# daovietanh190499/3D_Reconstruction

Measured on AMD Instinct MI355X. Metric: image-pairs matched/sec, higher is better.
Workload: dtype f32 descriptors: int8 MFMA certified filter + f64 re-score; 1 GPU; C3/C4 all-pairs BF-L2 + ratio 0.75: 257 imgs x 4096 kpts x 256-d, exact f32-input semantics (oracle.match.bf_match_exact, bit for bit); pairs=32896, api=dist.match_all_pairs_sharded(exact=True), match_mode=exact-float, parallelism=pairs/1

## Files before the change

### 3d_reconstruction_amd/csrc/match_exact.hip

```cpp
#include "match_dev.h"
#include "resolve_scratch.h"

namespace sfmhip {

__global__ __launch_bounds__(256) void desc_residual_kernel(const float* __restrict__ x, const int8_t* __restrict__ q,
                                                            int n_rows, int m_pad, int d, const int32_t* __restrict__ nk,
                                                            int mode, double* __restrict__ erow,
                                                            unsigned long long* __restrict__ eimg) {
    const int lane = threadIdx.x & 63;
    const int row = blockIdx.x * 4 + (threadIdx.x >> 6);
    if (row >= n_rows) return;
    const int img = row / m_pad, r = row % m_pad;
    if (r >= nk[img]) {
        if (lane == 0) erow[row] = 0.0;
        return;
    }
    const float* xr = x + (size_t)row * d;
    const int8_t* qr = q + (size_t)row * d;
    double s2 = 0.0, x2 = 0.0, v2 = 0.0;
    bool finite = true;
    for (int k = lane; k < d; k += 64) {
        const float xf = xr[k];
        const double xv = (double)xf;
        const double v = mode == 0 ? (double)((int)qr[k] + 128) : (double)qr[k] / 127.0;
        const double dl = xv - v;
        s2 = __builtin_fma(dl, dl, s2);
        x2 = __builtin_fma(xv, xv, x2);
        v2 = __builtin_fma(v, v, v2);
        finite = finite && __builtin_isfinite(xf);
    }
#pragma unroll
    for (int off = 32; off >= 1; off >>= 1) {
        s2 += __shfl_xor(s2, off);
        x2 += __shfl_xor(x2, off);
        v2 += __shfl_xor(v2, off);
    }
    const bool all_finite = __all(finite);
    if (lane == 0) {
        const double e = all_finite ? sqrt(s2) * (1.0 + 0x1p-40) + 0x1p-50 * (sqrt(x2) + sqrt(v2)) * (1.0 + 0x1p-40)
                                    : __builtin_inf();
        erow[row] = e;
        atomicMax(eimg + img, (unsigned long long)__double_as_longlong(e));
    }
}

constexpr int kResolveCap = 512;
#ifdef SFMHIP_RESOLVE_PROF
__device__ unsigned long long g_rprof[16];
#endif
template <int D, typename OutT>
__device__ __forceinline__ void resolve_row(int64_t e, int mark, const int8_t* __restrict__ q,
                                            const float* __restrict__ x, const int32_t* __restrict__ nk, int m_pad,
                                            const int32_t* __restrict__ pairs, const double* __restrict__ erow,
                                            const double* __restrict__ eimg, double s, double rn2, double rd2,
                                            OutT* __restrict__ m0, unsigned* __restrict__ n_resolved, float* sxa,
                                            int* sqa, int* scand, int lane) {
    constexpr int W4 = D / 4;
    const int pair = (int)(e / m_pad), i = (int)(e % m_pad);
    const int a = pairs[2 * pair], b = pairs[2 * pair + 1], nb = nk[b];
    const size_t arow = (size_t)a * m_pad + i;
    for (int k = lane; k < D; k += 64) sxa[k] = x[arow * D + k];
    for (int w = lane; w < W4; w += 64) sqa[w] = reinterpret_cast<const int*>(q + arow * D)[w];
    __builtin_amdgcn_fence(__ATOMIC_RELEASE, "wavefront");
    __builtin_amdgcn_wave_barrier();
    __builtin_amdgcn_fence(__ATOMIC_ACQUIRE, "wavefront");
    int na = 0;
    for (int w = lane; w < W4; w += 64) na = __builtin_amdgcn_sdot4(sqa[w], sqa[w], na, false);
#pragma unroll
    for (int off = 32; off >= 1; off >>= 1) na += __shfl_xor(na, off);
    const double se = (erow[arow] + eimg[b]) * s * (1.0 + 1e-12);
    const double bq = (se + (mark_sqrt_d2<OutT>(mark) + se) * (1.0 + 1e-12)) * (1.0 + 1e-12);
    const double tq = floor(bq * bq) + 1.0;
    int ncand = 0;
    for (int j0 = 0; j0 < nb; j0 += 64) {
        const int j = j0 + lane;
        bool in = false;
        if (j < nb) {
            const int4* qb = reinterpret_cast<const int4*>(q + ((size_t)b * m_pad + j) * D);
            int dot = 0, nbn = 0;
#pragma unroll 4
            for (int w4 = 0; w4 < W4 / 4; ++w4) {
                const int4 t = qb[w4];
                const int4 u = reinterpret_cast<const int4*>(sqa)[w4];
                dot = __builtin_amdgcn_sdot4(t.x, u.x, dot, false);
                dot = __builtin_amdgcn_sdot4(t.y, u.y, dot, false);
                dot = __builtin_amdgcn_sdot4(t.z, u.z, dot, false);
                dot = __builtin_amdgcn_sdot4(t.w, u.w, dot, false);
                nbn = __builtin_amdgcn_sdot4(t.x, t.x, nbn, false);
                nbn = __builtin_amdgcn_sdot4(t.y, t.y, nbn, false);
                nbn = __builtin_amdgcn_sdot4(t.z, t.z, nbn, false);
                nbn = __builtin_amdgcn_sdot4(t.w, t.w, nbn, false);
            }
            in = (double)((long long)na + nbn - 2LL * dot) <= tq;
        }
        const unsigned long long cb = __ballot(in);
        const int pos = ncand + __popcll(cb & ((1ull << lane) - 1ull));
        if (in && pos < kResolveCap) scand[pos] = j;
        ncand += __popcll(cb);
    }
    __builtin_amdgcn_fence(__ATOMIC_RELEASE, "wavefront");
    __builtin_amdgcn_wave_barrier();
    __builtin_amdgcn_fence(__ATOMIC_ACQUIRE, "wavefront");
    const bool every = ncand > kResolveCap;
    const int nc = every ? nb : ncand;
    double v1 = __builtin_inf(), v2 = __builtin_inf();
    int j1 = INT_MAX;
    for (int t = lane; t < nc; t += 64) {
        const int j = every ? t : scand[t];
        const float4* xb = reinterpret_cast<const float4*>(x + ((size_t)b * m_pad + j) * D);
        double acc = 0.0;
        for (int k4 = 0; k4 < D / 4; ++k4) {
            const float4 xv = xb[k4];
            double df;
            df = (double)sxa[4 * k4] - (double)xv.x;
            acc = acc + df * df;
            df = (double)sxa[4 * k4 + 1] - (double)xv.y;
            acc = acc + df * df;
            df = (double)sxa[4 * k4 + 2] - (double)xv.z;
            acc = acc + df * df;
            df = (double)sxa[4 * k4 + 3] - (double)xv.w;
            acc = acc + df * df;
        }
        if (acc < v1) { v2 = v1; v1 = acc; j1 = j; }
        else if (acc < v2) v2 = acc;
    }
#pragma unroll
    for (int off = 32; off >= 1; off >>= 1) {
        const double o1 = __shfl_xor(v1, off), o2 = __shfl_xor(v2, off);
        const int oj = __shfl_xor(j1, off);
        const bool mine = v1 < o1 || (v1 == o1 && j1 < oj);
        const double n2 = mine ? fmin(v2, o1) : fmin(o2, v1);
        if (!mine) { v1 = o1; j1 = oj; }
        v2 = n2;
    }
    const double p1 = rd2 * v1, e1 = __builtin_fma(rd2, v1, -p1);
    const double p2 = rn2 * v2, e2 = __builtin_fma(rn2, v2, -p2);
    const bool acc_ok = p1 < p2 || (p1 == p2 && e1 < e2);
    if (lane == 0) {
        m0[e] = (OutT)(acc_ok ? j1 : -1);
        if (n_resolved) atomicAdd(n_resolved, 1u);
    }
    __builtin_amdgcn_wave_barrier();
}

template <int D, typename OutT>
__global__ __launch_bounds__(256) void match_resolve_kernel(const int8_t* __restrict__ q, const float* __restrict__ x,
                                                            const int32_t* __restrict__ nk, int m_pad,
                                                            const int32_t* __restrict__ pairs, int P,
                                                            const double* __restrict__ erow,
                                                            const double* __restrict__ eimg, double s, double rn2,
                                                            double rd2, OutT* __restrict__ m0,
                                                            unsigned* __restrict__ n_resolved,
                                                            const unsigned* __restrict__ overflow = nullptr) {
    if (overflow && *overflow == 0u) return;
    constexpr int W4 = D / 4;
    __shared__ float sxa[4][D];
    __shared__ __attribute__((aligned(16))) int sqa[4][W4];
    __shared__ int scand[4][kResolveCap];
    const int lane = threadIdx.x & 63, wave = threadIdx.x >> 6;
    const int64_t total = (int64_t)P * m_pad;
    const int64_t nchunk = (total + 63) >> 6;
    for (int64_t c = (int64_t)blockIdx.x * 4 + wave; c < nchunk; c += (int64_t)gridDim.x * 4) {
        const int64_t e0 = c << 6;
        const int v = (e0 + lane < total) ? (int)m0[e0 + lane] : -1;
        unsigned long long bal = __ballot(v <= kUndecidedBase);
        while (bal) {
            const int l = __builtin_ctzll(bal);
            bal &= bal - 1;
            resolve_row<D, OutT>(e0 + l, __shfl(v, l), q, x, nk, m_pad, pairs, erow, eimg, s, rn2, rd2, m0, n_resolved,
                           sxa[wave], sqa[wave], scand[wave], lane);
        }
    }
}

template <typename OutT>
__global__ __launch_bounds__(256) void resolve_collect_kernel(const OutT* __restrict__ m0, int64_t total, int m_pad,
                                                              const int32_t* __restrict__ pairs,
                                                              unsigned* __restrict__ cnt, int64_t* __restrict__ list,
                                                              unsigned* __restrict__ overflow) {
    auto take = [&](int64_t e) {
        const int b = pairs[2 * (int)(e / m_pad) + 1];
        const unsigned slot = atomicAdd(cnt + b, 1u);
        if (slot < (unsigned)kResolveBucket) list[(size_t)b * kResolveBucket + slot] = e;
        else atomicOr(overflow, 1u);
    };
    constexpr int PER = 16 / sizeof(OutT);
    const int64_t n4 = total / PER;
    const int4* m4 = reinterpret_cast<const int4*>(m0);
    for (int64_t e4 = (int64_t)blockIdx.x * blockDim.x + threadIdx.x; e4 < n4; e4 += (int64_t)gridDim.x * blockDim.x) {
        const int4 v = m4[e4];
        if constexpr (sizeof(OutT) == 2) {
            const unsigned w[4] = {(unsigned)v.x, (unsigned)v.y, (unsigned)v.z, (unsigned)v.w};
            bool any = false;
#pragma unroll
            for (int h = 0; h < 4; ++h) {
                any |= (short)(w[h] & 0xFFFFu) <= kUndecidedBase;
                any |= (short)(w[h] >> 16) <= kUndecidedBase;
            }
            if (!any) continue;
#pragma unroll
            for (int h = 0; h < 4; ++h) {
                if ((short)(w[h] & 0xFFFFu) <= kUndecidedBase) take(PER * e4 + 2 * h);
                if ((short)(w[h] >> 16) <= kUndecidedBase) take(PER * e4 + 2 * h + 1);
            }
        } else {
            if (min(min(v.x, v.y), min(v.z, v.w)) > kUndecidedBase) continue;
            if (v.x <= kUndecidedBase) take(4 * e4);
            if (v.y <= kUndecidedBase) take(4 * e4 + 1);
            if (v.z <= kUndecidedBase) take(4 * e4 + 2);
            if (v.w <= kUndecidedBase) take(4 * e4 + 3);
        }
    }
}

__global__ __launch_bounds__(1024) void resolve_offsets_kernel(
    const unsigned* __restrict__ cnt, int n_img, unsigned* __restrict__ off, unsigned* __restrict__ okey,
    int* __restrict__ oimg, unsigned* __restrict__ xr, int* __restrict__ items, unsigned* __restrict__ ir,
    const unsigned* __restrict__ overflow) {
    __shared__ unsigned sr[1024], sk[1024];
    __shared__ unsigned sxs[9], sks[9];
    if (*overflow != 0u) return;
    const int tid = threadIdx.x;
    const int cap = n_img * (kResolveBucket / kResolveRows + 1);
    int ps[9];
    ps[0] = 0;
#pragma unroll
    for (int x = 0; x < 8; ++x) ps[x + 1] = ps[x] + (x < n_img ? (n_img - x + 7) / 8 : 0);
    unsigned carry_r = 0, carry_k = 0;
    for (int base = 0; base < n_img; base += 1024) {
        const int p = base + tid;
        int b = -1;
        unsigned cb = 0, ni = 0;
        if (p < n_img) {
            int x = 0;
#pragma unroll
            for (int y = 1; y < 8; ++y) x += (p >= ps[y]) ? 1 : 0;
            b = x + 8 * (p - ps[x]);
            cb = min(cnt[b], (unsigned)kResolveBucket);
            ni = (cb + kResolveRows - 1) / kResolveRows;
        }
        sr[tid] = cb;
        sk[tid] = ni;
        __syncthreads();
        for (int d = 1; d < 1024; d <<= 1) {
            const unsigned vr = tid >= d ? sr[tid - d] : 0u, vk = tid >= d ? sk[tid - d] : 0u;
            __syncthreads();
            sr[tid] += vr;
            sk[tid] += vk;
            __syncthreads();
        }
        const unsigned run = carry_r + sr[tid] - cb, k0 = carry_k + sk[tid] - ni;
        if (b >= 0) {
            off[b] = run;
            okey[p] = run;
            oimg[p] = b;
#pragma unroll
            for (int x = 0; x < 8; ++x)
                if (p == ps[x]) {
                    sxs[x] = run;
                    sks[x] = k0;
                }
            for (unsigned i = 0; i < ni; ++i) {
                items[k0 + i] = (int)(run + i * kResolveRows);
                items[cap + k0 + i] = (int)min((unsigned)kResolveRows, cb - i * kResolveRows);
                items[2 * cap + k0 + i] = b;
            }
        }
        carry_r += sr[1023];
        carry_k += sk[1023];
        __syncthreads();
    }
    if (tid < 9) {
        if (tid == 8 || ps[tid] >= n_img) {
            sxs[tid] = carry_r;
            sks[tid] = carry_k;
        }
    }
    __syncthreads();
    if (tid < 8) {
        xr[tid] = sxs[tid];
        xr[8 + tid] = sxs[tid + 1] - sxs[tid];
        ir[tid] = sks[tid];
        ir[8 + tid] = sks[tid + 1] - sks[tid];
    }
    if (tid == 0) okey[n_img] = carry_r;
}
__global__ __launch_bounds__(256) void resolve_flatten_kernel(const unsigned* __restrict__ okey,
                                                              const int* __restrict__ oimg, int n_img,
                                                              const int64_t* __restrict__ list,
                                                              int64_t* __restrict__ flat,
                                                              const unsigned* __restrict__ overflow) {
    if (*overflow != 0u) return;
    const unsigned total = okey[n_img];
    for (unsigned t = blockIdx.x * blockDim.x + threadIdx.x; t < total; t += gridDim.x * blockDim.x) {
        int lo = 0, hi = n_img - 1;
        while (lo < hi) {
            const int mid = (lo + hi + 1) >> 1;
            if (okey[mid] <= t) lo = mid;
            else hi = mid - 1;
        }
        flat[t] = list[(size_t)oimg[lo] * kResolveBucket + (t - okey[lo])];
    }
}

template <int D, typename OutT>
__global__ __launch_bounds__(256) void match_resolve_batched_kernel(
    const int8_t* __restrict__ q , const int32_t* __restrict__ norms,
    const float* __restrict__ x, const int32_t* __restrict__ nk, int m_pad,
    const int32_t* __restrict__ pairs, int n_img, const double* __restrict__ erow, const double* __restrict__ eimg,
    double s, double rn2, double rd2, OutT* __restrict__ m0, unsigned* __restrict__ n_resolved,
    const int64_t* __restrict__ flat, const int* __restrict__ items, const unsigned* __restrict__ ir,
    const unsigned* __restrict__ overflow) {
    constexpr int W4 = D / 4, R = kResolveRows;
    __shared__ __attribute__((aligned(16))) int sqa[R][W4];
    __shared__ float sxa[R][D];
    __shared__ int scand[R][kResolveCap];
    __shared__ int sncand[R], sna[R], sccd[R];
    __shared__ double stq[R];
    __shared__ int64_t se_[R];
    if (*overflow != 0u) return;
    const int tid = threadIdx.x, lane = tid & 63, wave = tid >> 6;
    const int cap = n_img * (kResolveBucket / kResolveRows + 1);
    const int xcd = blockIdx.x % 8, nx = (gridDim.x + 7 - xcd) / 8;
    const unsigned ib = ir[xcd], in = ir[8 + xcd];
    for (unsigned k = blockIdx.x / 8; k < in; k += nx) {
        const int f0 = items[ib + k], nr = items[cap + ib + k], b = items[2 * cap + ib + k];
        const int nb = nk[b];
        for (int t = tid; t < nr * W4; t += 256) {
            const int r = t / W4, w = t % W4;
            const int64_t e = flat[f0 + r];
            const size_t arow = (size_t)pairs[2 * (int)(e / m_pad)] * m_pad + (int)(e % m_pad);
            sqa[r][w] = reinterpret_cast<const int*>(q + arow * D)[w];
        }
        for (int t = tid; t < nr * D; t += 256) {
            const int r = t / D, kk = t % D;
            const int64_t e = flat[f0 + r];
            const size_t arow = (size_t)pairs[2 * (int)(e / m_pad)] * m_pad + (int)(e % m_pad);
            sxa[r][kk] = x[arow * D + kk];
        }
        if (tid < R) sncand[tid] = 0;
        __syncthreads();
        for (int r = wave; r < nr; r += 4) {
            int na = 0;
            for (int w = lane; w < W4; w += 64) na = __builtin_amdgcn_sdot4(sqa[r][w], sqa[r][w], na, false);
#pragma unroll
            for (int off = 32; off >= 1; off >>= 1) na += __shfl_xor(na, off);
            if (lane == 0) {
                const int64_t e = flat[f0 + r];
                const size_t arow = (size_t)pairs[2 * (int)(e / m_pad)] * m_pad + (int)(e % m_pad);
                const double se = (erow[arow] + eimg[b]) * s * (1.0 + 1e-12);
                const double bq = (se + (mark_sqrt_d2<OutT>((int)m0[e]) + se) * (1.0 + 1e-12)) * (1.0 + 1e-12);
                stq[r] = floor(bq * bq) + 1.0;
                sna[r] = na;
                sccd[r] = norms[arow] - na;
                se_[r] = e;
            }
        }
        __syncthreads();
        {
            using M16 = Mfma<16>;
            constexpr int KK = D / M16::KB;
            const int lr = lane & 15, grp = lane >> 4;
            i32x4 bqv[KK];
#pragma unroll
            for (int kk = 0; kk < KK; ++kk) bqv[kk] = *reinterpret_cast<const i32x4*>(&sqa[lr][kk * 16 + grp * 4]);
            const bool live = lr < nr;
            const long long na_r = live ? (long long)sna[lr] - sccd[lr] : 0;
            const double tq_r = live ? stq[lr] : -1.0;
            const size_t bbase = (size_t)b * m_pad;
            constexpr int TG = 4;
            for (int jg = wave * 16; jg < nb; jg += 64 * TG) {
                i32x4 av[TG][KK], nv[TG];
#pragma unroll
                for (int t = 0; t < TG; ++t) {
                    const int j0 = min(jg + 64 * t, m_pad - 16);
                    const int8_t* rp = q + (bbase + j0 + lr) * D + grp * 16;
#pragma unroll
                    for (int kk = 0; kk < KK; ++kk) av[t][kk] = *reinterpret_cast<const i32x4*>(rp + kk * M16::KB);
                    nv[t] = *reinterpret_cast<const i32x4*>(norms + bbase + j0 + 4 * grp);
                }
#pragma unroll
                for (int t = 0; t < TG; ++t) {
                    const int j0 = jg + 64 * t;
                    i32x4 acc = {0, 0, 0, 0};
#pragma unroll
                    for (int kk = 0; kk < KK; ++kk) acc = M16::run(av[t][kk], bqv[kk], acc);
#pragma unroll
                    for (int e = 0; e < 4; ++e) {
                        const int j = j0 + 4 * grp + e;
                        if (live && j < nb && (double)(na_r + nv[t][e] - 2LL * acc[e]) <= tq_r) {
                            const int pos = atomicAdd(&sncand[lr], 1);
                            if (pos < kResolveCap) scand[lr][pos] = j;
                        }
                    }
                }
            }
        }
        __syncthreads();
        for (int r = wave; r < nr; r += 4) {
            const int ncand = sncand[r];
            const bool every = ncand > kResolveCap;
#ifdef SFMHIP_RESOLVE_PROF
            if (lane == 0) {
                atomicAdd(&g_rprof[0], 1ull);
                atomicAdd(&g_rprof[1], (unsigned long long)ncand);
                if (every) atomicAdd(&g_rprof[2], 1ull);
                atomicMax(&g_rprof[3], (unsigned long long)ncand);
                atomicAdd(&g_rprof[4 + min(ncand / 64, 11)], 1ull);
            }
#endif
            const int nc = every ? nb : ncand;
            double v1 = __builtin_inf(), v2 = __builtin_inf();
            int j1 = INT_MAX;
            for (int t = lane; t < nc; t += 64) {
                const int j = every ? t : scand[r][t];
                const float4* xb = reinterpret_cast<const float4*>(x + ((size_t)b * m_pad + j) * D);
                double acc = 0.0;
                for (int k4 = 0; k4 < D / 4; ++k4) {
                    const float4 xv = xb[k4];
                    double df;
                    df = (double)sxa[r][4 * k4] - (double)xv.x;
                    acc = acc + df * df;
                    df = (double)sxa[r][4 * k4 + 1] - (double)xv.y;
                    acc = acc + df * df;
                    df = (double)sxa[r][4 * k4 + 2] - (double)xv.z;
                    acc = acc + df * df;
                    df = (double)sxa[r][4 * k4 + 3] - (double)xv.w;
                    acc = acc + df * df;
                }
                if (acc < v1 || (acc == v1 && j < j1)) { v2 = v1; v1 = acc; j1 = j; }
                else if (acc < v2) v2 = acc;
            }
#pragma unroll
            for (int off = 32; off >= 1; off >>= 1) {
                const double o1 = __shfl_xor(v1, off), o2 = __shfl_xor(v2, off);
                const int oj = __shfl_xor(j1, off);
                const bool mine = v1 < o1 || (v1 == o1 && j1 < oj);
                const double n2 = mine ? fmin(v2, o1) : fmin(o2, v1);
                if (!mine) { v1 = o1; j1 = oj; }
                v2 = n2;
            }
            const double p1 = rd2 * v1, e1 = __builtin_fma(rd2, v1, -p1);
            const double p2 = rn2 * v2, e2 = __builtin_fma(rn2, v2, -p2);
            const bool acc_ok = p1 < p2 || (p1 == p2 && e1 < e2);
            if (lane == 0) {
                m0[se_[r]] = (OutT)(acc_ok ? j1 : -1);
                if (n_resolved) atomicAdd(n_resolved, 1u);
            }
        }
        __syncthreads();
    }
}

struct ResolveLaunch {
    const int8_t* desc;
    const int32_t* norms;
    const int8_t* desc_q;
    const float* desc_f;
    const double *resid_row, *resid_img;
    const int32_t* n_kpts;
    int n_img, m_pad, d;
    const int32_t* pairs;
    int P;
    double s, rn2, rd2;
    uint32_t* n_resolved;
    int n_cu;
    char* scratch;
    ResolveScratch lay;
    hipStream_t stream;
    template <typename T> T* at(size_t off) const { return reinterpret_cast<T*>(scratch + off); }
};

template <int D, typename OutT>
static void launch_resolve_d(const ResolveLaunch& r, OutT* matches0) {
    int64_t *list = r.at<int64_t>(r.lay.list), *flat = r.at<int64_t>(r.lay.flat);
    unsigned *cnt = r.at<unsigned>(r.lay.cnt), *flag = r.at<unsigned>(r.lay.flag);
    unsigned *okey = r.at<unsigned>(r.lay.okey), *ir = r.at<unsigned>(r.lay.ir);
    int *oimg = r.at<int>(r.lay.oimg), *items = r.at<int>(r.lay.items);
    const int64_t total = (int64_t)r.P * r.m_pad;
    const int64_t nchunk = (total + 63) / 64;
    const int rgrid = (int)std::min<int64_t>((nchunk + 3) / 4, (int64_t)r.n_cu * 8);
    const int rxgrid = r.n_cu * 2;
    hipStream_t s = r.stream;
    hipLaunchKernelGGL(resolve_collect_kernel<OutT>, dim3(rgrid), dim3(256), 0, s, matches0, total, r.m_pad, r.pairs, cnt,
                       list, flag);
    hipLaunchKernelGGL(resolve_offsets_kernel, dim3(1), dim3(1024), 0, s, cnt, r.n_img, r.at<unsigned>(r.lay.off), okey,
                       oimg, r.at<unsigned>(r.lay.xr), items, ir, flag);
    hipLaunchKernelGGL(resolve_flatten_kernel, dim3(r.n_cu), dim3(256), 0, s, okey, oimg, r.n_img, list, flat, flag);
    hipLaunchKernelGGL((match_resolve_batched_kernel<D, OutT>), dim3(rxgrid), dim3(256), 0, s, r.desc, r.norms, r.desc_f,
                       r.n_kpts, r.m_pad, r.pairs, r.n_img, r.resid_row, r.resid_img, r.s, r.rn2, r.rd2, matches0,
                       r.n_resolved, flat, items, ir, flag);
    hipLaunchKernelGGL((match_resolve_kernel<D, OutT>), dim3(rgrid), dim3(256), 0, s, r.desc_q, r.desc_f, r.n_kpts,
                       r.m_pad, r.pairs, r.P, r.resid_row, r.resid_img, r.s, r.rn2, r.rd2, matches0, r.n_resolved, flag);
}

template <typename OutT>
int launch_resolve(const ResolveLaunch& r, OutT* matches0) {
    switch (r.d) {
        case 64: launch_resolve_d<64>(r, matches0); break;
        case 128: launch_resolve_d<128>(r, matches0); break;
        case 256: launch_resolve_d<256>(r, matches0); break;
        default: return SFMHIP_E_UNSUPPORTED;
    }
    return check_launch("match_resolve_kernel");
}
template int launch_resolve<int32_t>(const ResolveLaunch&, int32_t*);
template int launch_resolve<int16_t>(const ResolveLaunch&, int16_t*);

}

using namespace sfmhip;

#ifdef SFMHIP_RESOLVE_PROF
extern "C" int sfmhip_debug_resolve_prof(unsigned long long* out) {
    return hipMemcpyFromSymbol(out, HIP_SYMBOL(sfmhip::g_rprof), sizeof(unsigned long long) * 16) == hipSuccess ? 0 : -2;
}
#endif

extern "C" int sfmhip_desc_residual(const float* desc_f, const int8_t* desc_q, int n_img, int m_pad, int d,
                                    const int32_t* n_kpts, int mode, double* resid_row, double* resid_img,
                                    void* stream) {
    SFMHIP_REQUIRE(desc_f && desc_q && n_kpts && resid_row && resid_img, "sfmhip_desc_residual: null pointer");
    SFMHIP_REQUIRE(n_img > 0 && m_pad > 0 && d > 0, "sfmhip_desc_residual: bad shape");
    SFMHIP_REQUIRE(mode == 0 || mode == 1, "sfmhip_desc_residual: mode must be 0 or 1");
    const int64_t rows = (int64_t)n_img * m_pad;
    SFMHIP_REQUIRE(rows < INT_MAX, "sfmhip_desc_residual: too many rows");
    hipStream_t s = as_stream(stream);
    if (hipMemsetAsync(resid_img, 0, (size_t)n_img * sizeof(double), s) != hipSuccess) return check_launch("memset");
    hipLaunchKernelGGL(desc_residual_kernel, dim3(ceil_div(rows, 4)), dim3(256), 0, s, desc_f, desc_q, (int)rows, m_pad,
                       d, n_kpts, mode, resid_row, reinterpret_cast<unsigned long long*>(resid_img));
    return check_launch("desc_residual_kernel");
}

struct Fp6Bank {
    const uint8_t* dense;
    const int32_t* h;
    const float* hf;
};

template <typename OutT>
static int match_exact_impl(const int8_t* desc, const int32_t* norms, const int32_t* keys,
                            const int8_t* desc_q, const float* desc_f, const double* resid_row,
                            const double* resid_img, int mode, const int32_t* n_kpts, int n_img,
                            int m_pad, int d, const int32_t* pairs, int P, int ratio_num, int ratio_den,
                            OutT* matches0, int32_t* dist1, int32_t* dist2, uint32_t* n_resolved,
                            void* stream, const Fp6Bank* bank) {
    const uint8_t* dense = bank ? bank->dense : nullptr;
    const bool fp6 = dense && knobs().match_fp6 != 0;
    if (dense) {
        SFMHIP_REQUIRE(mode == 1 && !dist1 && !dist2 && (d == 128 || d == 256),
                       "sfmhip_match_pairs_exact_fp6: float mode, d in {128,256}, no distance outputs");
    }
    int n_iblk, nwg;
    if (int rc = check_match_call<OutT>(
            "sfmhip_match_pairs_exact", true, n_img, P, m_pad, mode, ratio_num, ratio_den,
            desc && norms && keys && desc_q && desc_f && resid_row && resid_img && n_kpts && pairs && matches0,
            fp6 ? kMatchFp6Rows : kMatchRows, &n_iblk, &nwg))
        return rc;
    if (P == 0) return SFMHIP_OK;
    hipStream_t s = as_stream(stream);
    if (n_resolved && hipMemsetAsync(n_resolved, 0, sizeof(uint32_t), s) != hipSuccess) return check_launch("memset");

    const ResolveScratch lay = resolve_scratch_layout(n_img, m_pad, !dist1 && !dist2, fp6, bank && bank->h);
    char* buf = nullptr;
    if (scratch_alloc(reinterpret_cast<void**>(&buf), lay.bytes, s) != hipSuccess) {
        (void)hipGetLastError();
        set_error("sfmhip_match_pairs_exact: scratch allocation failed");
        return SFMHIP_E_HIP;
    }
    if (hipMemsetAsync(buf + lay.cnt, 0, lay.off - lay.cnt, s) != hipSuccess) {
        scratch_free(buf, s);
        return check_launch("memset");
    }

    const long long rn2 = (long long)ratio_num * ratio_num, rd2 = (long long)ratio_den * ratio_den;
    const CertArgs ca{resid_row, resid_img, mode == 0 ? 1.0 : 1.0 / 127.0, knobs().match_cert == 0 ? 1 : 0};
    FilterLaunch f{desc, norms, bank && bank->h ? bank->h : keys, n_kpts, m_pad, d, pairs, n_iblk, nwg, rn2, rd2, ca, s,
                   dist1, dist2, dense, bank ? bank->hf : nullptr};
    if (lay.h_count) {
        int32_t* h = reinterpret_cast<int32_t*>(buf + lay.h);
        float* hf = fp6 ? reinterpret_cast<float*>(buf + lay.hf) : nullptr;
        launch_key_values(keys, (int64_t)lay.h_count, h, hf, s);
        f.keys = h;
        f.hf = hf;
    }
    int rc = fp6 ? launch_match_fp6(f, matches0) : launch_match_cert(f, matches0);

    if (rc == SFMHIP_OK) {
        const ResolveLaunch r{desc, norms, desc_q, desc_f, resid_row, resid_img, n_kpts, n_img, m_pad, d, pairs, P,
                              mode == 0 ? 1.0 : 127.0, (double)rn2, (double)rd2, n_resolved, cu_count(), buf, lay, s};
        rc = launch_resolve(r, matches0);
    }
    if (rc == SFMHIP_E_UNSUPPORTED) set_error("sfmhip_match_pairs_exact: descriptor dim %d not in {64,128,256}", d);
    scratch_free(buf, s);
    return rc;
}

extern "C" int sfmhip_match_pairs_exact(const int8_t* desc, const int32_t* norms, const int32_t* keys,
                                        const int8_t* desc_q, const float* desc_f, const double* resid_row,
                                        const double* resid_img, int mode, const int32_t* n_kpts, int n_img,
                                        int m_pad, int d, const int32_t* pairs, int P, int ratio_num, int ratio_den,
                                        int32_t* matches0, int32_t* dist1, int32_t* dist2, uint32_t* n_resolved,
                                        void* stream) {
    return match_exact_impl(desc, norms, keys, desc_q, desc_f, resid_row, resid_img, mode, n_kpts, n_img, m_pad, d,
                            pairs, P, ratio_num, ratio_den, matches0, dist1, dist2, n_resolved, stream, nullptr);
}

extern "C" int sfmhip_match_pairs_exact_i16(const int8_t* desc, const int32_t* norms, const int32_t* keys,
                                            const int8_t* desc_q, const float* desc_f, const double* resid_row,
                                            const double* resid_img, int mode, const int32_t* n_kpts, int n_img,
                                            int m_pad, int d, const int32_t* pairs, int P, int ratio_num,
                                            int ratio_den, int16_t* matches0, uint32_t* n_resolved, void* stream) {
    return match_exact_impl(desc, norms, keys, desc_q, desc_f, resid_row, resid_img, mode, n_kpts, n_img, m_pad, d,
                            pairs, P, ratio_num, ratio_den, matches0, (int32_t*)nullptr, (int32_t*)nullptr,
                            n_resolved, stream, nullptr);
}

extern "C" int sfmhip_match_pairs_exact_fp6(const uint8_t* dense, const int8_t* g, const int32_t* norms,
                                            const int32_t* keys, const float* desc_f, const double* resid_row,
                                            const double* resid_img, const int32_t* n_kpts, int n_img, int m_pad,
                                            int d, const int32_t* pairs, int P, int ratio_num, int ratio_den,
                                            int32_t* matches0, uint32_t* n_resolved, void* stream) {
    SFMHIP_REQUIRE(dense || P == 0, "sfmhip_match_pairs_exact_fp6: null pointer");
    const Fp6Bank bank{dense, nullptr, nullptr};
    return match_exact_impl(g, norms, keys, g, desc_f, resid_row, resid_img, 1, n_kpts, n_img, m_pad, d, pairs, P,
                            ratio_num, ratio_den, matches0, (int32_t*)nullptr, (int32_t*)nullptr, n_resolved, stream,
                            &bank);
}

extern "C" int sfmhip_match_pairs_exact_fp6_i16(const uint8_t* dense, const int8_t* g, const int32_t* norms,
                                                const int32_t* keys, const float* desc_f, const double* resid_row,
                                                const double* resid_img, const int32_t* n_kpts, int n_img, int m_pad,
                                                int d, const int32_t* pairs, int P, int ratio_num, int ratio_den,
                                                int16_t* matches0, uint32_t* n_resolved, void* stream) {
    SFMHIP_REQUIRE(dense || P == 0, "sfmhip_match_pairs_exact_fp6_i16: null pointer");
    const Fp6Bank bank{dense, nullptr, nullptr};
    return match_exact_impl(g, norms, keys, g, desc_f, resid_row, resid_img, 1, n_kpts, n_img, m_pad, d, pairs, P,
                            ratio_num, ratio_den, matches0, (int32_t*)nullptr, (int32_t*)nullptr, n_resolved, stream,
                            &bank);
}

extern "C" int sfmhip_match_pairs_exact_fp6_kv(const uint8_t* dense, const int8_t* g, const int32_t* norms,
                                               const int32_t* h, const float* hf, const float* desc_f,
                                               const double* resid_row, const double* resid_img, const int32_t* n_kpts,
                                               int n_img, int m_pad, int d, const int32_t* pairs, int P, int ratio_num,
                                               int ratio_den, int32_t* matches0, uint32_t* n_resolved, void* stream) {
    SFMHIP_REQUIRE((dense && hf) || P == 0, "sfmhip_match_pairs_exact_fp6_kv: null pointer");
    const Fp6Bank bank{dense, h, hf};
    return match_exact_impl(g, norms, h, g, desc_f, resid_row, resid_img, 1, n_kpts, n_img, m_pad, d, pairs, P,
                            ratio_num, ratio_den, matches0, (int32_t*)nullptr, (int32_t*)nullptr, n_resolved, stream,
                            &bank);
}

extern "C" int sfmhip_match_pairs_exact_fp6_kv_i16(const uint8_t* dense, const int8_t* g, const int32_t* norms,
                                                   const int32_t* h, const float* hf, const float* desc_f,
                                                   const double* resid_row, const double* resid_img,
                                                   const int32_t* n_kpts, int n_img, int m_pad, int d,
                                                   const int32_t* pairs, int P, int ratio_num, int ratio_den,
                                                   int16_t* matches0, uint32_t* n_resolved, void* stream) {
    SFMHIP_REQUIRE((dense && hf) || P == 0, "sfmhip_match_pairs_exact_fp6_kv_i16: null pointer");
    const Fp6Bank bank{dense, h, hf};
    return match_exact_impl(g, norms, h, g, desc_f, resid_row, resid_img, 1, n_kpts, n_img, m_pad, d, pairs, P,
                            ratio_num, ratio_den, matches0, (int32_t*)nullptr, (int32_t*)nullptr, n_resolved, stream,
                            &bank);
}
```

### 3d_reconstruction_amd/csrc/resolve_scratch.h

```cpp
#pragma once

#include <cstddef>
#include <cstdint>

namespace sfmhip {

constexpr int kResolveBucket = 4096;
constexpr int kResolveRows = 16;

struct ResolveScratch {
    size_t list;
    size_t cnt;
    size_t flag;
    size_t off;
    size_t okey;
    size_t oimg;
    size_t xr;
    size_t ir;
    size_t flat;
    size_t items;
    size_t h;
    size_t hf;
    size_t bytes;
    size_t h_count;
};

inline ResolveScratch resolve_scratch_layout(int n_img, int m_pad, bool value_only, bool fp6, bool has_bank_h) {
    const size_t n = (size_t)n_img, u = sizeof(unsigned);
    ResolveScratch r;
    r.list = 0;
    r.cnt = r.list + n * kResolveBucket * sizeof(int64_t);
    r.flag = r.cnt + n * u;
    r.off = r.flag + u;
    r.okey = r.off + n * u;
    r.oimg = r.okey + (n + 1) * u;
    r.xr = r.oimg + n * sizeof(int);
    r.ir = r.xr + 16 * u;
    r.flat = r.ir + 16 * u;
    r.items = r.flat + n * kResolveBucket * sizeof(int64_t);
    r.h = r.items + 3 * n * (kResolveBucket / kResolveRows + 1) * sizeof(int);
    r.h_count = value_only && !has_bank_h ? n * (size_t)m_pad : 0;
    r.hf = r.h + r.h_count * sizeof(int32_t);
    r.bytes = r.hf + (fp6 ? r.h_count * sizeof(float) : 0);
    return r;
}

}
```

Baseline: 634,300 pairs/s.

## Replace offsets/flatten/batched resolve with per-image multi-row resolve kernel

Removes the single-block prefix-scan offsets kernel and the flatten kernel. A new per-image resolve kernel distributes each image's undecided rows across blocks in 64-row units, read directly from the bucket list. It screens candidates with several 16-row MFMA tiles per loaded reference tile and can use FP6 dense operands when available. The exact f64 re-score is split across the whole block with a cross-wave top-2 merge. This cuts two launches and scratch traffic and reuses each reference tile across more query rows, at the cost of more registers and shared memory and a lower candidate cap per row.

```diff
diff --git a/3d_reconstruction_amd/csrc/match_exact.hip b/3d_reconstruction_amd/csrc/match_exact.hip
--- a/3d_reconstruction_amd/csrc/match_exact.hip
+++ b/3d_reconstruction_amd/csrc/match_exact.hip
@@ -213,248 +213,300 @@
     }
 }
 
-__global__ __launch_bounds__(1024) void resolve_offsets_kernel(
-    const unsigned* __restrict__ cnt, int n_img, unsigned* __restrict__ off, unsigned* __restrict__ okey,
-    int* __restrict__ oimg, unsigned* __restrict__ xr, int* __restrict__ items, unsigned* __restrict__ ir,
-    const unsigned* __restrict__ overflow) {
-    __shared__ unsigned sr[1024], sk[1024];
-    __shared__ unsigned sxs[9], sks[9];
-    if (*overflow != 0u) return;
-    const int tid = threadIdx.x;
-    const int cap = n_img * (kResolveBucket / kResolveRows + 1);
-    int ps[9];
-    ps[0] = 0;
-#pragma unroll
-    for (int x = 0; x < 8; ++x) ps[x + 1] = ps[x] + (x < n_img ? (n_img - x + 7) / 8 : 0);
-    unsigned carry_r = 0, carry_k = 0;
-    for (int base = 0; base < n_img; base += 1024) {
-        const int p = base + tid;
-        int b = -1;
-        unsigned cb = 0, ni = 0;
-        if (p < n_img) {
-            int x = 0;
-#pragma unroll
-            for (int y = 1; y < 8; ++y) x += (p >= ps[y]) ? 1 : 0;
-            b = x + 8 * (p - ps[x]);
-            cb = min(cnt[b], (unsigned)kResolveBucket);
-            ni = (cb + kResolveRows - 1) / kResolveRows;
-        }
-        sr[tid] = cb;
-        sk[tid] = ni;
-        __syncthreads();
-        for (int d = 1; d < 1024; d <<= 1) {
-            const unsigned vr = tid >= d ? sr[tid - d] : 0u, vk = tid >= d ? sk[tid - d] : 0u;
-            __syncthreads();
-            sr[tid] += vr;
-            sk[tid] += vk;
-            __syncthreads();
-        }
-        const unsigned run = carry_r + sr[tid] - cb, k0 = carry_k + sk[tid] - ni;
-        if (b >= 0) {
-            off[b] = run;
-            okey[p] = run;
-            oimg[p] = b;
-#pragma unroll
-            for (int x = 0; x < 8; ++x)
-                if (p == ps[x]) {
-                    sxs[x] = run;
-                    sks[x] = k0;
-                }
-            for (unsigned i = 0; i < ni; ++i) {
-                items[k0 + i] = (int)(run + i * kResolveRows);
-                items[cap + k0 + i] = (int)min((unsigned)kResolveRows, cb - i * kResolveRows);
-                items[2 * cap + k0 + i] = b;
-            }
-        }
-        carry_r += sr[1023];
-        carry_k += sk[1023];
-        __syncthreads();
-    }
-    if (tid < 9) {
-        if (tid == 8 || ps[tid] >= n_img) {
-            sxs[tid] = carry_r;
-            sks[tid] = carry_k;
-        }
-    }
-    __syncthreads();
-    if (tid < 8) {
-        xr[tid] = sxs[tid];
-        xr[8 + tid] = sxs[tid + 1] - sxs[tid];
-        ir[tid] = sks[tid];
-        ir[8 + tid] = sks[tid + 1] - sks[tid];
-    }
-    if (tid == 0) okey[n_img] = carry_r;
-}
-__global__ __launch_bounds__(256) void resolve_flatten_kernel(const unsigned* __restrict__ okey,
-                                                              const int* __restrict__ oimg, int n_img,
-                                                              const int64_t* __restrict__ list,
-                                                              int64_t* __restrict__ flat,
-                                                              const unsigned* __restrict__ overflow) {
-    if (*overflow != 0u) return;
-    const unsigned total = okey[n_img];
-    for (unsigned t = blockIdx.x * blockDim.x + threadIdx.x; t < total; t += gridDim.x * blockDim.x) {
-        int lo = 0, hi = n_img - 1;
-        while (lo < hi) {
-            const int mid = (lo + hi + 1) >> 1;
-            if (okey[mid] <= t) lo = mid;
-            else hi = mid - 1;
-        }
-        flat[t] = list[(size_t)oimg[lo] * kResolveBucket + (t - okey[lo])];
-    }
-}
-
-template <int D, typename OutT>
-__global__ __launch_bounds__(256) void match_resolve_batched_kernel(
-    const int8_t* __restrict__ q , const int32_t* __restrict__ norms,
-    const float* __restrict__ x, const int32_t* __restrict__ nk, int m_pad,
+__device__ __forceinline__ void wave_top2(double& v1, int& j1, double& v2) {
+#pragma unroll
+    for (int off = 32; off >= 1; off >>= 1) {
+        const double o1 = __shfl_xor(v1, off), o2 = __shfl_xor(v2, off);
+        const int oj = __shfl_xor(j1, off);
+        const bool mine = v1 < o1 || (v1 == o1 && j1 < oj);
+        const double n2 = mine ? fmin(v2, o1) : fmin(o2, v1);
+        if (!mine) { v1 = o1; j1 = oj; }
+        v2 = n2;
+    }
+}
+__device__ __forceinline__ bool ratio_accepts(double v1, double v2, double rn2, double rd2) {
+    const double p1 = rd2 * v1, e1 = __builtin_fma(rd2, v1, -p1);
+    const double p2 = rn2 * v2, e2 = __builtin_fma(rn2, v2, -p2);
+    return p1 < p2 || (p1 == p2 && e1 < e2);
+}
+
+template <int D, bool FP6> struct ResolveOperand;
+template <int D> struct ResolveOperand<D, true> {
+    static_assert(D % 128 == 0, "one FP6 MFMA takes 128 elements of k");
+    static constexpr int KK = D / 128, TG = D == 256 ? 6 : 8;
+    i32x4 lo;
+    i32x2 hi;
+    __device__ void load(const int8_t*, const uint8_t* dense, size_t row, int kk, int grp) {
+        const uint8_t* rp = dense + row * (3 * D / 4);
+        lo = *reinterpret_cast<const i32x4*>(rp + 16 * (kk * 4 + grp));
+        hi = *reinterpret_cast<const i32x2*>(rp + D / 2 + 8 * (kk * 4 + grp));
+    }
+    __device__ i32x8 tuple() const { return i32x8{lo[0], lo[1], lo[2], lo[3], hi[0], hi[1], 0, 0}; }
+    using acc_t = f32x4;
+    __device__ static acc_t run(const ResolveOperand& a, const ResolveOperand& b, acc_t c) {
+        return __builtin_amdgcn_mfma_scale_f32_16x16x128_f8f6f4(a.tuple(), b.tuple(), c, 2, 2, 0, 0, 0, 0);
+    }
+    __device__ static int dot(float v) { return (int)(64.f * v); }
+};
+template <int D> struct ResolveOperand<D, false> {
+    static constexpr int KK = D / 64, TG = 4;
+    i32x4 v;
+    __device__ void load(const int8_t* q, const uint8_t*, size_t row, int kk, int grp) {
+        v = *reinterpret_cast<const i32x4*>(q + row * D + kk * 64 + grp * 16);
+    }
+    using acc_t = i32x4;
+    __device__ static acc_t run(const ResolveOperand& a, const ResolveOperand& b, acc_t c) {
+        return Mfma<16>::run(a.v, b.v, c);
+    }
+    __device__ static int dot(int v) { return v; }
+};
+
+constexpr int kImageCap = 128;
+constexpr int kImageGroup = 4;
+
+template <int D, typename OutT, bool FP6>
+__global__ __launch_bounds__(256, 2) void match_resolve_image_kernel(
+    const int8_t* __restrict__ q , const uint8_t* __restrict__ dense,
+    const int32_t* __restrict__ norms, const float* __restrict__ x, const int32_t* __restrict__ nk, int m_pad,
     const int32_t* __restrict__ pairs, int n_img, const double* __restrict__ erow, const double* __restrict__ eimg,
     double s, double rn2, double rd2, OutT* __restrict__ m0, unsigned* __restrict__ n_resolved,
-    const int64_t* __restrict__ flat, const int* __restrict__ items, const unsigned* __restrict__ ir,
-    const unsigned* __restrict__ overflow) {
-    constexpr int W4 = D / 4, R = kResolveRows;
-    __shared__ __attribute__((aligned(16))) int sqa[R][W4];
-    __shared__ float sxa[R][D];
-    __shared__ int scand[R][kResolveCap];
-    __shared__ int sncand[R], sna[R], sccd[R];
-    __shared__ double stq[R];
-    __shared__ int64_t se_[R];
+    const int64_t* __restrict__ list, const unsigned* __restrict__ cnt, const unsigned* __restrict__ overflow) {
+    using Op = ResolveOperand<D, FP6>;
+    constexpr int T = kResolveRows, NS = T / 16, KK = Op::KK, TG = Op::TG, G = kImageGroup;
+    constexpr int PW = D + 2;
+    static_assert(T * 4 == 256 && T % 16 == 0, "four lanes stage a row");
+    __shared__ int scand[T][kImageCap];
+    __shared__ __attribute__((aligned(16))) double spb[4][G][PW];
+    __shared__ int sncand[T];
+    __shared__ long long snar[T];
+    __shared__ double stq[T];
+    __shared__ int64_t se_[T];
+    __shared__ size_t sarow[T];
+    __shared__ unsigned scnt[256];
+    __shared__ int sbig[T], snbig;
+    __shared__ double sw1[4], sw2[4];
+    __shared__ int swj[4];
     if (*overflow != 0u) return;
-    const int tid = threadIdx.x, lane = tid & 63, wave = tid >> 6;
-    const int cap = n_img * (kResolveBucket / kResolveRows + 1);
-    const int xcd = blockIdx.x % 8, nx = (gridDim.x + 7 - xcd) / 8;
-    const unsigned ib = ir[xcd], in = ir[8 + xcd];
-    for (unsigned k = blockIdx.x / 8; k < in; k += nx) {
-        const int f0 = items[ib + k], nr = items[cap + ib + k], b = items[2 * cap + ib + k];
-        const int nb = nk[b];
-        for (int t = tid; t < nr * W4; t += 256) {
-            const int r = t / W4, w = t % W4;
-            const int64_t e = flat[f0 + r];
-            const size_t arow = (size_t)pairs[2 * (int)(e / m_pad)] * m_pad + (int)(e % m_pad);
-            sqa[r][w] = reinterpret_cast<const int*>(q + arow * D)[w];
-        }
-        for (int t = tid; t < nr * D; t += 256) {
-            const int r = t / D, kk = t % D;
-            const int64_t e = flat[f0 + r];
-            const size_t arow = (size_t)pairs[2 * (int)(e / m_pad)] * m_pad + (int)(e % m_pad);
-            sxa[r][kk] = x[arow * D + kk];
-        }
-        if (tid < R) sncand[tid] = 0;
+    const int tid = threadIdx.x, lane = tid & 63, wave = __builtin_amdgcn_readfirstlane(tid >> 6);
+    const int lr = lane & 15, grp = lane >> 4;
+    const int xcd = blockIdx.x % 8, wx = blockIdx.x / 8, nx = (gridDim.x + 7 - xcd) / 8;
+    const int nix = xcd < n_img ? (n_img - xcd + 7) / 8 : 0;
+    unsigned unit = 0;
+    for (int c0 = 0; c0 < nix; c0 += 256) {
         __syncthreads();
-        for (int r = wave; r < nr; r += 4) {
-            int na = 0;
-            for (int w = lane; w < W4; w += 64) na = __builtin_amdgcn_sdot4(sqa[r][w], sqa[r][w], na, false);
-#pragma unroll
-            for (int off = 32; off >= 1; off >>= 1) na += __shfl_xor(na, off);
-            if (lane == 0) {
-                const int64_t e = flat[f0 + r];
-                const size_t arow = (size_t)pairs[2 * (int)(e / m_pad)] * m_pad + (int)(e % m_pad);
-                const double se = (erow[arow] + eimg[b]) * s * (1.0 + 1e-12);
-                const double bq = (se + (mark_sqrt_d2<OutT>((int)m0[e]) + se) * (1.0 + 1e-12)) * (1.0 + 1e-12);
-                stq[r] = floor(bq * bq) + 1.0;
-                sna[r] = na;
-                sccd[r] = norms[arow] - na;
-                se_[r] = e;
-            }
-        }
+        if (c0 + tid < nix) scnt[tid] = min(cnt[xcd + 8 * (c0 + tid)], (unsigned)kResolveBucket);
         __syncthreads();
-        {
-            using M16 = Mfma<16>;
-            constexpr int KK = D / M16::KB;
-            const int lr = lane & 15, grp = lane >> 4;
-            i32x4 bqv[KK];
-#pragma unroll
-            for (int kk = 0; kk < KK; ++kk) bqv[kk] = *reinterpret_cast<const i32x4*>(&sqa[lr][kk * 16 + grp * 4]);
-            const bool live = lr < nr;
-            const long long na_r = live ? (long long)sna[lr] - sccd[lr] : 0;
-            const double tq_r = live ? stq[lr] : -1.0;
-            const size_t bbase = (size_t)b * m_pad;
-            constexpr int TG = 4;
-            for (int jg = wave * 16; jg < nb; jg += 64 * TG) {
-                i32x4 av[TG][KK], nv[TG];
-#pragma unroll
-                for (int t = 0; t < TG; ++t) {
-                    const int j0 = min(jg + 64 * t, m_pad - 16);
-                    const int8_t* rp = q + (bbase + j0 + lr) * D + grp * 16;
-#pragma unroll
-                    for (int kk = 0; kk < KK; ++kk) av[t][kk] = *reinterpret_cast<const i32x4*>(rp + kk * M16::KB);
-                    nv[t] = *reinterpret_cast<const i32x4*>(norms + bbase + j0 + 4 * grp);
+        const int cn = min(256, nix - c0);
+        for (int ci = 0; ci < cn; ++ci) {
+            const unsigned n = __builtin_amdgcn_readfirstlane(scnt[ci]), np = (n + T - 1) / T;
+            const unsigned unit0 = unit;
+            unit += np;
+            for (unsigned p = ((unsigned)wx + nx - unit0 % nx) % nx; p < np; p += nx) {
+                const int b = xcd + 8 * (c0 + ci), nb = nk[b];
+                const size_t bbase = (size_t)b * m_pad;
+                const unsigned each = n / np, rem = n % np;
+                const unsigned first = p * each + min(p, rem);
+                const int nr = (int)(each + (p < rem ? 1u : 0u));
+                {
+                    const int r = tid >> 2, part = tid & 3;
+                    int na = 0;
+                    int64_t e = 0;
+                    size_t arow = 0;
+                    if (r < nr) {
+                        e = list[(size_t)b * kResolveBucket + first + r];
+                        arow = (size_t)pairs[2 * (int)(e / m_pad)] * m_pad + (int)(e % m_pad);
+                        const int* qa = reinterpret_cast<const int*>(q + arow * D) + part * (D / 16);
+#pragma unroll
+                        for (int w = 0; w < D / 16; ++w) na = __builtin_amdgcn_sdot4(qa[w], qa[w], na, false);
+                    }
+                    na += __shfl_xor(na, 1);
+                    na += __shfl_xor(na, 2);
+                    if (r < nr && part == 0) {
+                        const double se = (erow[arow] + eimg[b]) * s * (1.0 + 1e-12);
+                        const double bq = (se + (mark_sqrt_d2<OutT>((int)m0[e]) + se) * (1.0 + 1e-12)) * (1.0 + 1e-12);
+                        stq[r] = floor(bq * bq) + 1.0;
+                        snar[r] = 2LL * na - norms[arow];
+                        se_[r] = e;
+                        sarow[r] = arow;
+                    }
+                    if (tid < T) sncand[tid] = 0;
+                    if (tid == 0) snbig = 0;
                 }
-#pragma unroll
-                for (int t = 0; t < TG; ++t) {
-                    const int j0 = jg + 64 * t;
-                    i32x4 acc = {0, 0, 0, 0};
-#pragma unroll
-                    for (int kk = 0; kk < KK; ++kk) acc = M16::run(av[t][kk], bqv[kk], acc);
-#pragma unroll
-                    for (int e = 0; e < 4; ++e) {
-                        const int j = j0 + 4 * grp + e;
-                        if (live && j < nb && (double)(na_r + nv[t][e] - 2LL * acc[e]) <= tq_r) {
-                            const int pos = atomicAdd(&sncand[lr], 1);
-                            if (pos < kResolveCap) scand[lr][pos] = j;
+                __syncthreads();
+                {
+                    Op bq[NS][KK];
+                    long long na_r[NS];
+                    double tq_r[NS];
+                    const int ns = (nr + 15) >> 4;
+#pragma unroll
+                    for (int t = 0; t < NS; ++t) {
+                        const int r = 16 * t + lr;
+                        const bool live = r < nr;
+                        const size_t ar = sarow[live ? r : 0];
+                        na_r[t] = live ? snar[r] : 0;
+                        tq_r[t] = live ? stq[r] : -1.0;
+#pragma unroll
+                        for (int kk = 0; kk < KK; ++kk) bq[t][kk].load(q, dense, ar, kk, grp);
+                    }
+                    const int ntile = (nb + 15) >> 4;
+                    for (int t0 = wave; t0 < ntile; t0 += 4 * TG) {
+                        Op av[TG][KK];
+                        i32x4 nv[TG];
+#pragma unroll
+                        for (int t = 0; t < TG; ++t) {
+                            const int j0 = min((t0 + 4 * t) * 16, m_pad - 16);
+#pragma unroll
+                            for (int kk = 0; kk < KK; ++kk) av[t][kk].load(q, dense, bbase + j0 + lr, kk, grp);
+                            nv[t] = *reinterpret_cast<const i32x4*>(norms + bbase + j0 + 4 * grp);
+                        }
+#pragma unroll
+                        for (int t = 0; t < TG; ++t) {
+                            const int j0 = (t0 + 4 * t) * 16;
+                            if (j0 >= nb) continue;
+#pragma unroll
+                            for (int rt = 0; rt < NS; ++rt) {
+                                if (rt >= ns) continue;
+                                typename Op::acc_t acc = {0, 0, 0, 0};
+#pragma unroll
+                                for (int kk = 0; kk < KK; ++kk) acc = Op::run(av[t][kk], bq[rt][kk], acc);
+#pragma unroll
+                                for (int e = 0; e < 4; ++e) {
+                                    const int j = j0 + 4 * grp + e;
+                                    if (j < nb && (double)(na_r[rt] + nv[t][e] - 2LL * Op::dot(acc[e])) <= tq_r[rt]) {
+                                        const int pos = atomicAdd(&sncand[16 * rt + lr], 1);
+                                        if (pos < kImageCap) scand[16 * rt + lr][pos] = j;
+                                    }
+                                }
+                            }
                         }
                     }
                 }
+                __syncthreads();
+                {
+                    constexpr int LPC = D / 4, CPI = 64 / LPC, NIT = G / CPI;
+                    static_assert(CPI * NIT == G, "a group is whole wave loads");
+                    const int k4 = lane % LPC, csub = lane / LPC;
+                    double(*pb)[PW] = spb[wave];
+                    for (int r = wave; r < nr; r += 4) {
+                        const int ncand = sncand[r];
+#ifdef SFMHIP_RESOLVE_PROF
+                        if (lane == 0) {
+                            atomicAdd(&g_rprof[0], 1ull);
+                            atomicAdd(&g_rprof[1], (unsigned long long)ncand);
+                            if (ncand > kImageCap) atomicAdd(&g_rprof[2], 1ull);
+                            atomicMax(&g_rprof[3], (unsigned long long)ncand);
+                            atomicAdd(&g_rprof[4 + min(ncand / 64, 11)], 1ull);
+                        }
+#endif
+                        if (ncand > kImageCap) {
+                            if (lane == 0) sbig[atomicAdd(&snbig, 1)] = r;
+                            continue;
+                        }
+                        const float4 xa = *reinterpret_cast<const float4*>(x + sarow[r] * D + 4 * k4);
+                        double v1 = __builtin_inf(), v2 = __builtin_inf();
+                        int j1 = INT_MAX;
+                        for (int g0 = 0; g0 < ncand; g0 += G) {
+                            float4 xv[NIT];
+#pragma unroll
+                            for (int it = 0; it < NIT; ++it) {
+                                const int j = scand[r][min(g0 + it * CPI + csub, ncand - 1)];
+                                xv[it] = *reinterpret_cast<const float4*>(x + (bbase + j) * D + 4 * k4);
+                            }
+#pragma unroll
+                            for (int it = 0; it < NIT; ++it) {
+                                double* pp = &pb[it * CPI + csub][4 * k4];
+                                double df;
+                                df = (double)xa.x - (double)xv[it].x;
+                                pp[0] = df * df;
+                                df = (double)xa.y - (double)xv[it].y;
+                                pp[1] = df * df;
+                                df = (double)xa.z - (double)xv[it].z;
+                                pp[2] = df * df;
+                                df = (double)xa.w - (double)xv[it].w;
+                                pp[3] = df * df;
+                            }
+                            __builtin_amdgcn_fence(__ATOMIC_RELEASE, "wavefront");
+                            __builtin_amdgcn_wave_barrier();
+                            __builtin_amdgcn_fence(__ATOMIC_ACQUIRE, "wavefront");
+                            if (lane < G && g0 + lane < ncand) {
+                                const double* pp = pb[lane];
+                                double acc = 0.0;
+#pragma unroll 16
+                                for (int k = 0; k < D; ++k) acc = acc + pp[k];
+                                const int j = scand[r][g0 + lane];
+                                if (acc < v1 || (acc == v1 && j < j1)) { v2 = v1; v1 = acc; j1 = j; }
+                                else if (acc < v2) v2 = acc;
+                            }
+                            __builtin_amdgcn_fence(__ATOMIC_RELEASE, "wavefront");
+                            __builtin_amdgcn_wave_barrier();
+                            __builtin_amdgcn_fence(__ATOMIC_ACQUIRE, "wavefront");
+                        }
+                        wave_top2(v1, j1, v2);
+                        if (lane == 0) {
+                            m0[se_[r]] = (OutT)(ratio_accepts(v1, v2, rn2, rd2) ? j1 : -1);
+                            if (n_resolved) atomicAdd(n_resolved, 1u);
+                        }
+                    }
+                }
+                __syncthreads();
+                const int nbig = __builtin_amdgcn_readfirstlane(snbig);
+                for (int bi = 0; bi < nbig; ++bi) {
+                    const int r = sbig[bi];
+                    float* sx = reinterpret_cast<float*>(&spb[0][0][0]);
+                    for (int k = tid; k < D; k += 256) sx[k] = x[sarow[r] * D + k];
+                    __syncthreads();
+                    double v1 = __builtin_inf(), v2 = __builtin_inf();
+                    int j1 = INT_MAX;
+                    for (int j = tid; j < nb; j += 256) {
+                        const float4* xb = reinterpret_cast<const float4*>(x + (bbase + j) * D);
+                        double acc = 0.0;
+#pragma unroll 16
+                        for (int k4 = 0; k4 < D / 4; ++k4) {
+                            const float4 xv = xb[k4];
+                            double df;
+                            df = (double)sx[4 * k4] - (double)xv.x;
+                            acc = acc + df * df;
+                            df = (double)sx[4 * k4 + 1] - (double)xv.y;
+                            acc = acc + df * df;
+                            df = (double)sx[4 * k4 + 2] - (double)xv.z;
+                            acc = acc + df * df;
+                            df = (double)sx[4 * k4 + 3] - (double)xv.w;
+                            acc = acc + df * df;
+                        }
+                        if (acc < v1) { v2 = v1; v1 = acc; j1 = j; }
+                        else if (acc < v2) v2 = acc;
+                    }
+                    wave_top2(v1, j1, v2);
+                    if (lane == 0) {
+                        sw1[wave] = v1;
+                        sw2[wave] = v2;
+                        swj[wave] = j1;
+                    }
+                    __syncthreads();
+                    if (tid == 0) {
+                        for (int w = 1; w < 4; ++w) {
+                            const double o1 = sw1[w], o2 = sw2[w];
+                            const int oj = swj[w];
+                            const bool mine = v1 < o1 || (v1 == o1 && j1 < oj);
+                            const double n2 = mine ? fmin(v2, o1) : fmin(o2, v1);
+                            if (!mine) { v1 = o1; j1 = oj; }
+                            v2 = n2;
+                        }
+                        m0[se_[r]] = (OutT)(ratio_accepts(v1, v2, rn2, rd2) ? j1 : -1);
+                        if (n_resolved) atomicAdd(n_resolved, 1u);
+                    }
+                    __syncthreads();
+                }
+                __syncthreads();
             }
         }
-        __syncthreads();
-        for (int r = wave; r < nr; r += 4) {
-            const int ncand = sncand[r];
-            const bool every = ncand > kResolveCap;
-#ifdef SFMHIP_RESOLVE_PROF
-            if (lane == 0) {
-                atomicAdd(&g_rprof[0], 1ull);
-                atomicAdd(&g_rprof[1], (unsigned long long)ncand);
-                if (every) atomicAdd(&g_rprof[2], 1ull);
-                atomicMax(&g_rprof[3], (unsigned long long)ncand);
-                atomicAdd(&g_rprof[4 + min(ncand / 64, 11)], 1ull);
-            }
-#endif
-            const int nc = every ? nb : ncand;
-            double v1 = __builtin_inf(), v2 = __builtin_inf();
-            int j1 = INT_MAX;
-            for (int t = lane; t < nc; t += 64) {
-                const int j = every ? t : scand[r][t];
-                const float4* xb = reinterpret_cast<const float4*>(x + ((size_t)b * m_pad + j) * D);
-                double acc = 0.0;
-                for (int k4 = 0; k4 < D / 4; ++k4) {
-                    const float4 xv = xb[k4];
-                    double df;
-                    df = (double)sxa[r][4 * k4] - (double)xv.x;
-                    acc = acc + df * df;
-                    df = (double)sxa[r][4 * k4 + 1] - (double)xv.y;
-                    acc = acc + df * df;
-                    df = (double)sxa[r][4 * k4 + 2] - (double)xv.z;
-                    acc = acc + df * df;
-                    df = (double)sxa[r][4 * k4 + 3] - (double)xv.w;
-                    acc = acc + df * df;
-                }
-                if (acc < v1 || (acc == v1 && j < j1)) { v2 = v1; v1 = acc; j1 = j; }
-                else if (acc < v2) v2 = acc;
-            }
-#pragma unroll
-            for (int off = 32; off >= 1; off >>= 1) {
-                const double o1 = __shfl_xor(v1, off), o2 = __shfl_xor(v2, off);
-                const int oj = __shfl_xor(j1, off);
-                const bool mine = v1 < o1 || (v1 == o1 && j1 < oj);
-                const double n2 = mine ? fmin(v2, o1) : fmin(o2, v1);
-                if (!mine) { v1 = o1; j1 = oj; }
-                v2 = n2;
-            }
-            const double p1 = rd2 * v1, e1 = __builtin_fma(rd2, v1, -p1);
-            const double p2 = rn2 * v2, e2 = __builtin_fma(rn2, v2, -p2);
-            const bool acc_ok = p1 < p2 || (p1 == p2 && e1 < e2);
-            if (lane == 0) {
-                m0[se_[r]] = (OutT)(acc_ok ? j1 : -1);
-                if (n_resolved) atomicAdd(n_resolved, 1u);
-            }
-        }
-        __syncthreads();
     }
 }
 
 struct ResolveLaunch {
     const int8_t* desc;
     const int32_t* norms;
+    const uint8_t* dense;
     const int8_t* desc_q;
     const float* desc_f;
     const double *resid_row, *resid_img;
@@ -473,10 +525,8 @@
 
 template <int D, typename OutT>
 static void launch_resolve_d(const ResolveLaunch& r, OutT* matches0) {
-    int64_t *list = r.at<int64_t>(r.lay.list), *flat = r.at<int64_t>(r.lay.flat);
+    int64_t* list = r.at<int64_t>(r.lay.list);
     unsigned *cnt = r.at<unsigned>(r.lay.cnt), *flag = r.at<unsigned>(r.lay.flag);
-    unsigned *okey = r.at<unsigned>(r.lay.okey), *ir = r.at<unsigned>(r.lay.ir);
-    int *oimg = r.at<int>(r.lay.oimg), *items = r.at<int>(r.lay.items);
     const int64_t total = (int64_t)r.P * r.m_pad;
     const int64_t nchunk = (total + 63) / 64;
     const int rgrid = (int)std::min<int64_t>((nchunk + 3) / 4, (int64_t)r.n_cu * 8);
@@ -484,12 +534,17 @@
     hipStream_t s = r.stream;
     hipLaunchKernelGGL(resolve_collect_kernel<OutT>, dim3(rgrid), dim3(256), 0, s, matches0, total, r.m_pad, r.pairs, cnt,
                        list, flag);
-    hipLaunchKernelGGL(resolve_offsets_kernel, dim3(1), dim3(1024), 0, s, cnt, r.n_img, r.at<unsigned>(r.lay.off), okey,
-                       oimg, r.at<unsigned>(r.lay.xr), items, ir, flag);
-    hipLaunchKernelGGL(resolve_flatten_kernel, dim3(r.n_cu), dim3(256), 0, s, okey, oimg, r.n_img, list, flat, flag);
-    hipLaunchKernelGGL((match_resolve_batched_kernel<D, OutT>), dim3(rxgrid), dim3(256), 0, s, r.desc, r.norms, r.desc_f,
-                       r.n_kpts, r.m_pad, r.pairs, r.n_img, r.resid_row, r.resid_img, r.s, r.rn2, r.rd2, matches0,
-                       r.n_resolved, flat, items, ir, flag);
+    auto image = [&](auto kern) {
+        hipLaunchKernelGGL(kern, dim3(rxgrid), dim3(256), 0, s, r.desc, r.dense, r.norms, r.desc_f, r.n_kpts, r.m_pad,
+                           r.pairs, r.n_img, r.resid_row, r.resid_img, r.s, r.rn2, r.rd2, matches0, r.n_resolved, list,
+                           cnt, flag);
+    };
+    if constexpr (D % 128 == 0) {
+        if (r.dense) image(match_resolve_image_kernel<D, OutT, true>);
+        else image(match_resolve_image_kernel<D, OutT, false>);
+    } else {
+        image(match_resolve_image_kernel<D, OutT, false>);
+    }
     hipLaunchKernelGGL((match_resolve_kernel<D, OutT>), dim3(rgrid), dim3(256), 0, s, r.desc_q, r.desc_f, r.n_kpts,
                        r.m_pad, r.pairs, r.P, r.resid_row, r.resid_img, r.s, r.rn2, r.rd2, matches0, r.n_resolved, flag);
 }
@@ -568,7 +623,7 @@
         set_error("sfmhip_match_pairs_exact: scratch allocation failed");
         return SFMHIP_E_HIP;
     }
-    if (hipMemsetAsync(buf + lay.cnt, 0, lay.off - lay.cnt, s) != hipSuccess) {
+    if (hipMemsetAsync(buf + lay.cnt, 0, lay.h - lay.cnt, s) != hipSuccess) {
         scratch_free(buf, s);
         return check_launch("memset");
     }
@@ -587,7 +642,7 @@
     int rc = fp6 ? launch_match_fp6(f, matches0) : launch_match_cert(f, matches0);
 
     if (rc == SFMHIP_OK) {
-        const ResolveLaunch r{desc, norms, desc_q, desc_f, resid_row, resid_img, n_kpts, n_img, m_pad, d, pairs, P,
+        const ResolveLaunch r{desc, norms, dense, desc_q, desc_f, resid_row, resid_img, n_kpts, n_img, m_pad, d, pairs, P,
                               mode == 0 ? 1.0 : 127.0, (double)rn2, (double)rd2, n_resolved, cu_count(), buf, lay, s};
         rc = launch_resolve(r, matches0);
     }
diff --git a/3d_reconstruction_amd/csrc/resolve_scratch.h b/3d_reconstruction_amd/csrc/resolve_scratch.h
--- a/3d_reconstruction_amd/csrc/resolve_scratch.h
+++ b/3d_reconstruction_amd/csrc/resolve_scratch.h
@@ -6,19 +6,12 @@
 namespace sfmhip {
 
 constexpr int kResolveBucket = 4096;
-constexpr int kResolveRows = 16;
+constexpr int kResolveRows = 64;
 
 struct ResolveScratch {
     size_t list;
     size_t cnt;
     size_t flag;
-    size_t off;
-    size_t okey;
-    size_t oimg;
-    size_t xr;
-    size_t ir;
-    size_t flat;
-    size_t items;
     size_t h;
     size_t hf;
     size_t bytes;
@@ -31,14 +24,7 @@
     r.list = 0;
     r.cnt = r.list + n * kResolveBucket * sizeof(int64_t);
     r.flag = r.cnt + n * u;
-    r.off = r.flag + u;
-    r.okey = r.off + n * u;
-    r.oimg = r.okey + (n + 1) * u;
-    r.xr = r.oimg + n * sizeof(int);
-    r.ir = r.xr + 16 * u;
-    r.flat = r.ir + 16 * u;
-    r.items = r.flat + n * kResolveBucket * sizeof(int64_t);
-    r.h = r.items + 3 * n * (kResolveBucket / kResolveRows + 1) * sizeof(int);
+    r.h = (r.flag + u + 255) / 256 * 256;
     r.h_count = value_only && !has_bank_h ? n * (size_t)m_pad : 0;
     r.hf = r.h + r.h_count * sizeof(int32_t);
     r.bytes = r.hf + (fp6 ? r.h_count * sizeof(float) : 0);
```

Result: no change. 639,200 pairs/s, median of 6 (+0.8%).
